# vpc-ccg/circminer

Measured on AMD Instinct MI355X. Metric: paired reads/sec (whole node), hg38 k=20, 2x150 bp; circ_report bit-exact, higher is better.
Workload: dtype int32/u8 (chain scores f64)

## Files before the change

### circminer_amd/csrc/cm_hot.hip

```cpp
#include <chrono>
#include <hip/hip_runtime.h>
#include <rocprim/device/device_radix_sort.hpp>

#include <algorithm>
#include <atomic>
#include <cstdarg>
#include <cstdio>
#include <cstdlib>
#include <cstring>
#include <string>
#include <functional>
#include <thread>
#include <vector>

#include "circminer_hot.h"
#include "cm_core.h"
#include "cm_aos.h"
#include "cm_index_build.h"

using cmc::Core;
using cmc::KCore;

namespace {

constexpr int MAX_SLOTS = 16;
constexpr uint32_t TILE_PAIRS = 1u << 20;
constexpr uint32_t TILE_PAIRS_MAX = 1u << 21;
constexpr int BLK = 256;
constexpr int BLK_CHAIN = 64;
#include "cm_dp_engine.h"

enum ProfClass { PC_NONE = -1, PC_SEED = 0, PC_CHAIN = 1, PC_PAIR = 2, PC_SCAN = 3, PC_HEAVY = 4, PC_ORDER = 5, PC_CHAIN_HEAVY = 6, PC_PREFETCH = 7, PC_COUNT = 8 };
enum Counter {
    CN_PROBES = 0 , CN_PAIR_ROUNDS = 3, CN_RERUN = 4 ,
    CN_FALL = 5, CN_FALL_2ND = 6,
    CN_CD_LANE = 8, CN_CD_PHASE = 13, CN_CD_WAVE = 16, CN_CD_EVENTS = 20, CN_CD_LEVELS = 21, CN_CD_PROBLEMS = 22, CN_CD_PASSES = 23, CN_CD_CELLS = 24,
    CN_CD_REGLOG = 25, CN_CD_BATCHES = 26, CN_CD_PRE_USED = 27, CN_CD_PRE_UNUSED = 28,
    CN_HP_ATTEMPT = 8, CN_HP_STRIDE = 8, CN_HP_UNPAIRED = 24, CN_HP_CHAINS = 25, CN_HP_SEQ_TASKS = 26, CN_HP_EARLY = 27, CN_HP_EARLY_FIRST = 28,
    CN_WORDS = 32
};
static_assert(CN_CD_CELLS < CN_WORDS && CN_HP_EARLY_FIRST < CN_WORDS && CN_HP_ATTEMPT + CN_HP_STRIDE + 5 < CN_HP_UNPAIRED, "d_counters has CN_WORDS words");
enum Pin {
    PIN_COLLECT_N = 0, PIN_COLLECT_ERR = 1,
    PIN_DEV_ERR = 0,
    PIN_POOL_ERR = 2,
    PIN_HEAVY_LOAD = 4,
    PIN_CELLS = 8,
    PIN_RERUN_N = 12, PIN_FALL_N = 14,
    PIN_WORDS = 16
};
constexpr size_t PIN_BYTES = PIN_WORDS * sizeof(unsigned long long);
static_assert(PIN_BYTES == 128 && PIN_FALL_N + 1 < PIN_WORDS && PIN_CELLS + 3 < PIN_RERUN_N, "the landing zone has 16 words");
struct ReadsDev {
    const uint8_t *seq1, *seq2;
    const uint64_t *off1, *off2;
};

__global__ void __launch_bounds__(BLK) k_seed(KCore kc, ReadsDev rd, const uint8_t *active, uint64_t pair0, uint32_t n_tile, int S,
                                              uint32_t *sstart, uint32_t *scnt, uint32_t *sraw, unsigned long long *counters) {
    const Core c = cmc::to_core(kc);
    __shared__ unsigned int sh[3];
    if (threadIdx.x < 3) sh[threadIdx.x] = 0;
    __syncthreads();
    const uint64_t q = (uint64_t)blockIdx.x * BLK + threadIdx.x;
    const uint64_t total = (uint64_t)n_tile * 4u * (uint64_t)S;
    if (q < total) {
        const uint32_t s = (uint32_t)(q % (uint64_t)S);
// ... 1827 lines not shown
struct StreamDef {
    hipStream_t Streams::*st;
    const char *name;
    StreamKind kind;
};
constexpr StreamDef STREAMS[] = {
    {&Streams::B, "main", BLOCKING},           {&Streams::B2, "heavy chains", BLOCKING},     {&Streams::C, "copy", NON_BLOCKING},
    {&Streams::P, "pairs", NON_BLOCKING_LOWEST}, {&Streams::P2, "heavy pairs", NON_BLOCKING}, {&Streams::R, "re-run", NON_BLOCKING},
    {&Streams::O, "pair ordering", NON_BLOCKING}, {&Streams::S, "seeding", NON_BLOCKING},
};
struct Events {
    hipEvent_t fork = nullptr, join = nullptr;
    hipEvent_t join_p = nullptr, tail = nullptr;
    hipEvent_t flags = nullptr;
    hipEvent_t staged = nullptr, retired = nullptr;
    hipEvent_t order[2] = {nullptr, nullptr};
    hipEvent_t seed[2] = {nullptr, nullptr};
    hipEvent_t first[2] = {nullptr, nullptr};
    hipEvent_t prep[2] = {nullptr, nullptr}, pair[2] = {nullptr, nullptr};
    hipEvent_t *begin() { return &fork; }
    hipEvent_t *end() { return begin() + sizeof(Events) / sizeof(hipEvent_t); }
};
static_assert(sizeof(Events) == 17 * sizeof(hipEvent_t), "Events holds events only");

}

struct cm_ctx {
    cm_params P{};
    unsigned id = 0;
    int teardown_errors = 0;
    Streams st;
    Events ev;
    std::vector<DevMem *> bufs[2];
    struct Rerun {
        bool deferred = false;
        cmc::KCore core;
        ReadsDev rd;
        uint64_t p0 = 0;
        uint32_t nt = 0;
        cm_chain *chains = nullptr;
        int32_t *nchain = nullptr, *high = nullptr;
        uint8_t *act_out = nullptr;
        int is_last = 0, cap2 = 0;
        size_t lds2 = 0;
        bool fall = false;
        size_t lds_heavy = 0;
        int str_cap = 0;
        unsigned fall_grid = 0;
    } rerun[2];
    bool pair_pending[2] = {false, false};
    int item_base = 0;
    bool pre_launched = false;
    bool pre_ready = false;
    int pre_slot = -1, pre_b = 0;
    uint64_t pre_gen = 0, pre_n = 0;
    uint32_t pre_nt = 0;
    BatchBuf<uint8_t> d_ones;
    uint64_t ones_cap = 0;
    unsigned long long *h_pin = nullptr;
    uint32_t h_pin_nt = 0;
    std::string err = "";
    Slot slots[MAX_SLOTS];
    uint64_t n_pairs = 0;
    ReadBufs rd;
    BatchBuf<cm_mapped_read> d_state;
    BatchBuf<uint8_t> d_active;
    BatchBuf<uint8_t> d_active_b;
    BatchBuf<int32_t> d_cat;
    int n_seeds = 0, max_len = 0;
    bool staged = false;
    uint64_t st_n_pairs = 0;
    ReadBufs st_rd;
    BatchBuf<cm_mapped_read> st_prior;
    bool st_has_prior = false;
    int st_max_len = 0;
    uint32_t tile = 0;
    SeedSet seed[2];
    ChainRecs rec[2];
    PairSetMem pair_mem;
    PairSet pset[2];
    PairSort sort;
    ChainWork dp;
    HeavyPipe hp;
    Collect col;
    BatchBuf<unsigned long long> d_lane_clk;
    BatchBuf<HRes> d_hres;
    BatchBuf<unsigned long long> d_type_hist;
    BatchBuf<unsigned long long> d_heavy_load;
    BatchBuf<cmc::MemoSpill> d_spill;
    CtxBuf<unsigned long long> d_pool_cursor;
    unsigned long long *pool_cursor(int s) const { return d_pool_cursor + s; }
    CtxBuf<int> d_err;
    CtxBuf<unsigned long long> d_counters;
    std::vector<unsigned long long> h_celloff;
    bool prof = false;
// ... 58 lines not shown
    m.cap = bytes;
    if (!m.listed) (m.listed = &c->bufs[L])->push_back(&m);
    return e;
}
void release(cm_ctx *c, Life l) {
    for (DevMem *m : c->bufs[l]) {
        dfree(c, *m);
        m->listed = nullptr;
    }
    c->bufs[l].clear();
}

void free_reads(cm_ctx *c) {
    if (c->st.C) report_hip(c, "hipStreamSynchronize(copy stream)", hipStreamSynchronize(c->st.C));
    release(c, BATCH);
    c->pset[0] = c->pset[1] = PairSet{};
    c->ones_cap = 0;
    c->pre_launched = c->pre_ready = false;
    c->staged = false;
    c->st_n_pairs = 0;
    c->n_pairs = 0;
    c->tile = 0;
}

static hipEvent_t take_event(cm_ctx *c) {
    hipEvent_t e = nullptr;
    if (!c->ev_free.empty()) {
        e = c->ev_free.back();
        c->ev_free.pop_back();
    } else (void)hipEventCreate(&e);
    return e;
}
struct Timer {
// ... 63 lines not shown
    if (!ctx->slots[slot].loaded) return fail(ctx, CM_ESTATE, "contig slot %d not loaded", slot);
    if (need_annot && !ctx->slots[slot].has_annot) return fail(ctx, CM_ESTATE, "annotation of slot %d not loaded", slot);
    return CM_OK;
}

ReadsDev reads_dev(const ReadBufs &r) { return ReadsDev{r.seq1_base + cmc::CM_STAGE_PAD, r.seq2_base + cmc::CM_STAGE_PAD, r.off1, r.off2}; }
ReadsDev current_reads(const cm_ctx *ctx) { return reads_dev(ctx->rd); }

constexpr unsigned HP_PLAN_GRID = 2048;
static bool heavy_pipeline() {
    static const bool v = !(getenv("CM_HEAVY_PIPELINE") && getenv("CM_HEAVY_PIPELINE")[0] == '0');
    return v;
}
static unsigned long long chain_light_w() {
    static const unsigned long long v = getenv("CM_CHAIN_LIGHT_W") ? strtoull(getenv("CM_CHAIN_LIGHT_W"), nullptr, 10) : 256ull;
    return v;
}
static unsigned int chain_light_cells() {
    static const unsigned int v = getenv("CM_CHAIN_LIGHT_CELLS") ? (unsigned)atoi(getenv("CM_CHAIN_LIGHT_CELLS")) : 96u;
    return v;
}

static int seed_classes(cm_ctx *ctx, uint64_t pair0, uint32_t n_tile, const uint8_t *act, int s, hipStream_t st, const ChainRecs *rb, bool defer = false) {
    const int S = ctx->n_seeds;
    const uint32_t n_prob = n_tile * 4u;
    if ((uint64_t)n_prob * (uint64_t)S == 0) return CM_OK;
    const SeedSet &sb = ctx->seed[s];
    Timer t(ctx, PC_ORDER, st);
    launch(ctx, PC_ORDER, k_chain_cls, dim3((n_prob + BLK - 1) / BLK), dim3(BLK), 0, st, sb.scnt, sb.sraw, S, n_prob, sb.cls4, defer ? sb.thigh : rb->high,
           chain_light_w(), chain_light_cells(), defer ? (int32_t *)nullptr : rb->nchain, defer ? (uint16_t *)nullptr : rb->resid, act, pair0);
// ... 753 lines not shown
    ctx->tile = tile;
    const size_t nprob = (size_t)tile * 4, nprobe = nprob * (size_t)(ctx->n_seeds ? ctx->n_seeds : 1);
    for (SeedSet &sd : ctx->seed) {
        HIPCHK(ctx, ensure(ctx, sd.sstart, nprobe * 4));
        HIPCHK(ctx, ensure(ctx, sd.scnt, nprobe * 4));
        HIPCHK(ctx, ensure(ctx, sd.sraw, nprobe * 4));
        HIPCHK(ctx, ensure(ctx, sd.celloff, (nprob + 2) * 8));
        HIPCHK(ctx, ensure(ctx, sd.bmax, (nprob / SCAN_ELEMS + 2) * 4));
        HIPCHK(ctx, ensure(ctx, sd.bsum, (nprob / SCAN_ELEMS + 2) * 8));
        HIPCHK(ctx, ensure(ctx, sd.cctr, CTR_WORDS * sizeof(unsigned int)));
        HIPCHK(ctx, ensure(ctx, sd.cblk, (size_t)N_CLS * (4 * (size_t)tile / CLS_T + 2) * sizeof(unsigned int)));
        HIPCHK(ctx, ensure(ctx, sd.cls4, (size_t)tile * 4));
        HIPCHK(ctx, ensure(ctx, sd.perm4, (size_t)tile * 4 * 4));
        HIPCHK(ctx, ensure(ctx, sd.thigh, (size_t)tile * 4 * sizeof(int32_t)));
    }
    for (ChainRecs &cr : ctx->rec) {
        HIPCHK(ctx, ensure(ctx, cr.chains, nprob * CM_BESTCHAINLIM * sizeof(cm_chain)));
        HIPCHK(ctx, ensure(ctx, cr.nchain, nprob * 4));
        HIPCHK(ctx, ensure(ctx, cr.high, nprob * 4));
        HIPCHK(ctx, ensure(ctx, cr.resid, (size_t)tile * 4 * sizeof(uint16_t)));
    }
    unsigned long long cap = (unsigned long long)nprob * 64ull;
    const unsigned long long worst = (unsigned long long)ctx->P.seed_lim * (unsigned long long)(ctx->n_seeds ? ctx->n_seeds : 1);
    if (cap < (8ull << 20)) cap = 8ull << 20;
    if (cap < worst) cap = worst;
    if (cap > ctx->dp.cells_cap || !ctx->dp.score) ctx->dp.cells_cap = cap;
    HIPCHK(ctx, ensure(ctx, ctx->dp.score, ctx->dp.cells_cap * sizeof(double)));
    HIPCHK(ctx, ensure(ctx, ctx->dp.prev, ctx->dp.cells_cap * sizeof(int32_t)));
    HIPCHK(ctx, ensure(ctx, ctx->sort.cls, (size_t)tile));
    PairSetMem &pm = ctx->pair_mem;
    HIPCHK(ctx, ensure(ctx, pm.perm, (size_t)tile * 4 * 2));
    HIPCHK(ctx, ensure(ctx, pm.hlist, (size_t)tile * 4 * 2));
    HIPCHK(ctx, ensure(ctx, ctx->d_hres, (size_t)HEAVY_GRID_MAX * (64 * sizeof(HRes) + HEAVY_SCRATCH)));
    if (heavy_pipeline()) {
        const size_t tc = getenv("CM_HP_TASKS_CAP") ? (size_t)std::max(1, atoi(getenv("CM_HP_TASKS_CAP"))) : std::max<size_t>((size_t)tile * 6, 4096);
        const size_t uc = getenv("CM_HP_UNP_CAP") ? (size_t)std::max(1, atoi(getenv("CM_HP_UNP_CAP"))) : std::max<size_t>((size_t)tile * 4, 4096);
        ctx->hp.tasks_cap = (uint32_t)tc;
        ctx->hp.unp_cap = (uint32_t)uc;
        HIPCHK(ctx, ensure(ctx, ctx->hp.pairs, (size_t)tile * sizeof(HPair)));
        HIPCHK(ctx, ensure(ctx, ctx->hp.list2, (size_t)tile * 4));
        HIPCHK(ctx, ensure(ctx, pm.hp_fall, (size_t)tile * 4 * 2));
        HIPCHK(ctx, ensure(ctx, pm.hp_fallctr, 2 * sizeof(unsigned int)));
        HIPCHK(ctx, ensure(ctx, ctx->hp.T, tc * sizeof(HTask)));
        HIPCHK(ctx, ensure(ctx, ctx->hp.tcls, tc));
        HIPCHK(ctx, ensure(ctx, ctx->hp.tperm, tc * 4));
        HIPCHK(ctx, ensure(ctx, ctx->hp.tblk, (size_t)N_CLS * (tc / CLS_T + 2) * sizeof(unsigned int)));
        HIPCHK(ctx, ensure(ctx, ctx->hp.tctr, CTR_WORDS * sizeof(unsigned int)));
        HIPCHK(ctx, ensure(ctx, ctx->hp.pre, tc * 4 * sizeof(cmc::PreDP)));
        HIPCHK(ctx, ensure(ctx, ctx->hp.q, tc * 4 * 4));
        HIPCHK(ctx, ensure(ctx, ctx->hp.res, tc * sizeof(HRes)));
        HIPCHK(ctx, ensure(ctx, ctx->hp.U, uc * sizeof(HUnp)));
        HIPCHK(ctx, ensure(ctx, ctx->hp.pre2, uc * 2 * sizeof(cmc::PreDP)));
        HIPCHK(ctx, ensure(ctx, ctx->hp.q2, uc * 2 * 4));
        HIPCHK(ctx, ensure(ctx, ctx->hp.lists, (size_t)HP_PLAN_GRID * HEAVY_LIST * 2));
        HIPCHK(ctx, ensure(ctx, ctx->hp.ctr, HC_WORDS * sizeof(unsigned int)));
    }
    {
        const uint32_t *before = pm.pair_err;
        HIPCHK(ctx, ensure(ctx, pm.pair_err, (size_t)tile * 4 * 2));
        if (pm.pair_err != before) HIPCHK(ctx, hipMemsetAsync(pm.pair_err, 0, (size_t)tile * 4 * 2, ctx->st.P));
    }
    HIPCHK(ctx, ensure(ctx, pm.retry_list, (size_t)tile * 4 * 2));
    HIPCHK(ctx, ensure(ctx, pm.retry_ctr, 4 * sizeof(unsigned int)));
    HIPCHK(ctx, ensure(ctx, ctx->d_heavy_load, sizeof(unsigned long long)));
    HIPCHK(ctx, ensure(ctx, ctx->d_spill, (size_t)RETRY_GRID * BLK_PAIR * RETRY_SPILL * sizeof(cmc::MemoSpill)));
    HIPCHK(ctx, ensure(ctx, pm.cls_ctr, 2 * CTR_WORDS * sizeof(unsigned int)));
    HIPCHK(ctx, ensure(ctx, ctx->sort.ctr2, CTR_WORDS * sizeof(unsigned int)));
    HIPCHK(ctx, ensure(ctx, ctx->sort.sub, (size_t)tile));
    HIPCHK(ctx, ensure(ctx, ctx->sort.perm1, (size_t)tile * 4));
    HIPCHK(ctx, ensure(ctx, ctx->sort.ctr3, CTR_WORDS * sizeof(unsigned int)));
    HIPCHK(ctx, ensure(ctx, ctx->sort.sub2, (size_t)tile));
    HIPCHK(ctx, ensure(ctx, ctx->sort.perm0, (size_t)tile * 4));
    HIPCHK(ctx, ensure(ctx, ctx->sort.blk_cnt, (size_t)N_CLS * (4 * (size_t)tile / CLS_T + 2) * sizeof(unsigned int)));
    if (getenv("CM_LANE_CLK")) {
#if defined(CM_DIAG)
        const size_t clk_words = 16 * 2 + 1;
#else
        const size_t clk_words = 1;
#endif
        HIPCHK(ctx, ensure(ctx, ctx->d_lane_clk, n * 8 * clk_words));
        HIPCHK(ctx, hipMemsetAsync(ctx->d_lane_clk, 0, n * 8 * clk_words, ctx->st.B));
    }
    unsigned long long pool = (unsigned long long)nprob * 2048ull;
    if (pool < (256ull << 20)) pool = 256ull << 20;
    if (pool > (8ull << 30)) pool = 8ull << 30;
    if (const char *e = getenv("CM_POOL_BYTES")) {
        const unsigned long long v = strtoull(e, nullptr, 10);
        if (v >= 4096 && !ctx->dp.pool) pool = v;
    }
    if (pool > ctx->dp.pool_bytes || !ctx->dp.pool) ctx->dp.pool_bytes = pool;
    HIPCHK(ctx, ensure(ctx, ctx->dp.pool, ctx->dp.pool_bytes));
    for (int b = 0; b < 2; ++b) {
        const size_t at = (size_t)b * tile;
        ctx->pset[b] = PairSet{pm.perm + at,       pm.hlist + at,      pm.cls_ctr + (size_t)b * CTR_WORDS,
                               pm.pair_err + at,   pm.retry_list + at, pm.retry_ctr + 2 * b,
                               pm.hp_fall ? pm.hp_fall + at : nullptr, pm.hp_fallctr ? pm.hp_fallctr + b : nullptr};
    }
    return CM_OK;
}

static int copy_reads(cm_ctx *ctx, const cm_reads *rd, hipStream_t st, ReadBufs &to) {
    const uint64_t n = rd->n_pairs;
    const size_t b1 = (size_t)rd->off1[n] - (size_t)rd->off1[0], b2 = (size_t)rd->off2[n] - (size_t)rd->off2[0];
    if (rd->off1[0] != 0 || rd->off2[0] != 0) return fail(ctx, CM_EINVAL, "read offsets must start at 0");
    const size_t pad = cmc::CM_STAGE_PAD;
    HIPCHK(ctx, ensure(ctx, to.seq1_base, b1 + 2 * pad));
    HIPCHK(ctx, ensure(ctx, to.seq2_base, b2 + 2 * pad));
// ... 3 lines not shown
    HIPCHK(ctx, hipMemsetAsync(to.seq1_base + pad + b1, 0, pad, st));
    HIPCHK(ctx, hipMemsetAsync(to.seq2_base, 0, pad, st));
    HIPCHK(ctx, hipMemsetAsync(to.seq2_base + pad + b2, 0, pad, st));
    if (b1) HIPCHK(ctx, hipMemcpyAsync(to.seq1_base + pad, rd->seq1, b1, hipMemcpyHostToDevice, st));
    if (b2) HIPCHK(ctx, hipMemcpyAsync(to.seq2_base + pad, rd->seq2, b2, hipMemcpyHostToDevice, st));
    HIPCHK(ctx, hipMemcpyAsync(to.off1, rd->off1, (n + 1) * sizeof(uint64_t), hipMemcpyHostToDevice, st));
    HIPCHK(ctx, hipMemcpyAsync(to.off2, rd->off2, (n + 1) * sizeof(uint64_t), hipMemcpyHostToDevice, st));
    return CM_OK;
}

int cm_reads_upload(cm_ctx *ctx, const cm_reads *rd, const cm_mapped_read *prior) {
    if (!ctx || !rd) return CM_EINVAL;
    HIPCHK(ctx, hipSetDevice(ctx->P.device));
    HIPCHK(ctx, hipStreamSynchronize(ctx->st.B));
    const uint64_t n = rd->n_pairs;
    ctx->pre_ready = false;
    ctx->n_pairs = 0;
    ctx->tile = 0;
    if (n == 0) {
        free_reads(ctx);
        return CM_OK;
    }
    int max_len = 0;
    int rc = check_reads(ctx, rd, &max_len);
    if (rc) return rc;
    if ((rc = copy_reads(ctx, rd, ctx->st.B, ctx->rd))) return rc;
    if ((rc = prepare_resident(ctx, n, max_len))) return rc;
    ctx->n_pairs = n;
    KCore k{};
    k.P = ctx->P;
    hipLaunchKernelGGL(k_init_state, dim3((unsigned)((n + BLK - 1) / BLK)), dim3(BLK), 0, ctx->st.B, k, ctx->d_state, ctx->d_active, ctx->d_cat, n);
// ... 1 lines not shown
        HIPCHK(ctx, hipMemcpyAsync(ctx->d_state, prior, n * sizeof(cm_mapped_read), hipMemcpyHostToDevice, ctx->st.B));
    }
    HIPCHK(ctx, hipStreamSynchronize(ctx->st.B));
    return CM_OK;
}

int cm_reads_stage(cm_ctx *ctx, const cm_reads *rd, const cm_mapped_read *prior) {
    if (!ctx || !rd) return CM_EINVAL;
    HIPCHK(ctx, hipSetDevice(ctx->P.device));
    if (rd->n_pairs == 0) return fail(ctx, CM_EINVAL, "cm_reads_stage: empty batch");
    int max_len = 0;
    int rc = check_reads(ctx, rd, &max_len);
    if (rc) return rc;
    HIPCHK(ctx, hipStreamSynchronize(ctx->st.C));
    ctx->staged = false;
    ctx->pre_launched = false;
    if ((rc = copy_reads(ctx, rd, ctx->st.C, ctx->st_rd))) return rc;
    ctx->st_has_prior = prior != nullptr;
    if (prior) {
        HIPCHK(ctx, ensure(ctx, ctx->st_prior, rd->n_pairs * sizeof(cm_mapped_read)));
        HIPCHK(ctx, hipMemcpyAsync(ctx->st_prior, prior, rd->n_pairs * sizeof(cm_mapped_read), hipMemcpyHostToDevice, ctx->st.C));
    }
    HIPCHK(ctx, hipEventRecord(ctx->ev.staged, ctx->st.C));
    ctx->st_n_pairs = rd->n_pairs;
    ctx->st_max_len = max_len;
    ctx->staged = true;
    return CM_OK;
}

int cm_reads_swap(cm_ctx *ctx) {
    if (!ctx) return CM_EINVAL;
    HIPCHK(ctx, hipSetDevice(ctx->P.device));
    if (!ctx->staged) return fail(ctx, CM_ESTATE, "cm_reads_swap: no staged batch");
    swap(ctx->rd, ctx->st_rd);
    ctx->staged = false;
    const uint64_t n = ctx->st_n_pairs;
    ctx->pre_ready = ctx->pre_launched;
    ctx->pre_launched = false;
    ctx->pre_n = n;
    ctx->n_pairs = 0;
    int rc = prepare_resident(ctx, n, ctx->st_max_len);
    if (rc) return rc;
    ctx->n_pairs = n;
    HIPCHK(ctx, hipStreamWaitEvent(ctx->st.B, ctx->ev.staged, 0));
    KCore k{};
    k.P = ctx->P;
    hipLaunchKernelGGL(k_init_state, dim3((unsigned)((n + BLK - 1) / BLK)), dim3(BLK), 0, ctx->st.B, k, ctx->d_state, ctx->d_active, ctx->d_cat, n);
    if (ctx->st_has_prior)
        HIPCHK(ctx, hipMemcpyAsync(ctx->d_state, ctx->st_prior, n * sizeof(cm_mapped_read), hipMemcpyDeviceToDevice, ctx->st.B));
    HIPCHK(ctx, hipEventRecord(ctx->ev.retired, ctx->st.B));
    HIPCHK(ctx, hipStreamWaitEvent(ctx->st.C, ctx->ev.retired, 0));
    HIPCHK(ctx, hipGetLastError());
    return CM_OK;
// ... 26 lines not shown
    bool fell = false;
    if (ctx->rerun[b].fall && (!wait || *(const volatile unsigned int *)(ctx->h_pin + PIN_FALL_N + b) != 0u)) {
        const int rc = launch_fall_back(ctx, b, ctx->st.R);
        if (rc) return rc;
        fell = true;
    }
    if (!wait || fell || *(const volatile unsigned int *)(ctx->h_pin + PIN_RERUN_N + b) != 0u) {
        const int rc = launch_rerun(ctx, b);
        if (rc) return rc;
    }
    HIPCHK(ctx, hipEventRecord(ctx->ev.pair[b], ctx->st.R));
    return CM_OK;
}

static int run_pair_tile(cm_ctx *ctx, const KCore &core, uint64_t p0, uint32_t nt, int is_last_round, const uint8_t *act_in, uint8_t *act_out,
                         const ChainRecs &rb, int b, bool same_tile_as_prev, bool defer) {
    const ReadsDev rd = current_reads(ctx);
    hipStream_t sp = ctx->st.P, sp2 = ctx->st.P2, sp3 = ctx->st.R;
    {
        int rc;
        if ((rc = settle_pair(ctx, b))) return rc;
        if (same_tile_as_prev && (rc = settle_pair(ctx, b ^ 1))) return rc;
    }
    hipStream_t so = ctx->st.O;
    HIPCHK(ctx, hipStreamWaitEvent(so, ctx->ev.prep[b], 0));
    if (same_tile_as_prev && ctx->pair_pending[b ^ 1]) HIPCHK(ctx, hipStreamWaitEvent(so, ctx->ev.pair[b ^ 1], 0));
    const PairSet &ps = ctx->pset[b];
    uint32_t *const perm = ps.perm, *const hlist = ps.hlist, *const pair_err = ps.pair_err;
    unsigned int *const cls_ctr = ps.cls_ctr, *const retry_ctr = ps.retry_ctr;
    constexpr int str_slack = 4;
    const int str_cap = ((ctx->max_len - ctx->P.kmer + ctx->P.band + str_slack + 7) / 8) * 8;
    constexpr unsigned slots_per_simd = 4;
    const size_t lds_bytes = (size_t)2 * lbuf_bytes(str_cap) * BLK_PAIR;
    const size_t lds_heavy = lds_bytes + HG * sizeof(HSlot);
    const int cap2 = std::min(((2 * ctx->max_len + 64 + 7) / 8) * 8, 1016);
    const size_t lds2 = (size_t)2 * lbuf_bytes(cap2) * BLK_PAIR;
    {
        static std::atomic<size_t> lim[3] = {{48u * 1024u}, {48u * 1024u}, {48u * 1024u}};
        const void *fn[3] = {(const void *)k_pair, (const void *)k_pair_rerun, (const void *)k_pair_heavy};
        const size_t want[3] = {lds_bytes, lds2, lds_heavy};
        for (int k = 0; k < 3; ++k)
// ... 137 lines not shown
    struct Item { uint64_t p0; uint32_t nt; int r; };
    std::vector<Item> items;
    const uint64_t n_tiles = (ctx->n_pairs + ctx->tile - 1) / ctx->tile;
    const bool round_major = n_tiles >= 2;
    auto tile_nt = [&](uint64_t t) { return (uint32_t)((ctx->n_pairs - t * ctx->tile < ctx->tile) ? ctx->n_pairs - t * ctx->tile : ctx->tile); };
    if (round_major) {
        for (int r = 0; r < n_rounds; ++r)
            for (uint64_t t = 0; t < n_tiles; ++t) items.push_back(Item{t * ctx->tile, tile_nt(t), r});
    } else {
        for (uint64_t t = 0; t < n_tiles; ++t)
            for (int r = 0; r < n_rounds; ++r) items.push_back(Item{t * ctx->tile, tile_nt(t), r});
    }
    const int n_items = (int)items.size();
    std::vector<int> tiles_of_round((size_t)n_rounds, 0);
    const bool use_pre = ctx->pre_ready && slots[0] == ctx->pre_slot && ctx->slots[slots[0]].gen == ctx->pre_gen && ctx->n_pairs == ctx->pre_n &&
                         items[0].nt == ctx->pre_nt && (ctx->item_base & 1) == ctx->pre_b;
    ctx->pre_ready = ctx->pre_launched = false;
    if (use_pre) ++ctx->launches[PC_PREFETCH];
    const ReadsDev rd_cur = current_reads(ctx);
    auto prep_flags = [&](int i) -> const uint8_t * {
        const int r = items[i].r;
        return round_major ? A[r & 1] : ((r == 0) ? A[0] : A[(r - 1) & 1]);
    };
    std::vector<char> seeded((size_t)n_items, 0);
    bool pre_seeded = false;
    const bool early_ok = round_major;
    auto issue_seed_early = [&](int i) -> int {
        HIPCHK(ctx, hipStreamWaitEvent(ctx->st.S, ctx->ev.flags, 0));
        if (n_tiles == 2 && i >= 2) HIPCHK(ctx, hipStreamWaitEvent(ctx->st.S, ctx->ev.first[(ctx->item_base + i) & 1], 0));
        const ChainRecs &rbe = ctx->rec[(ctx->item_base + i) & 1];
        const int e = run_seed_tile(ctx, make_core(ctx, ctx->slots[slots[items[i].r]]), rd_cur, items[i].p0, items[i].nt, prep_flags(i), i & 1, ctx->st.S, &rbe, true);
        seeded[(size_t)i] = 1;
        return e;
    };
    auto issue_seed = [&](int i, hipStream_t st) -> int {
        const int b = (ctx->item_base + i) & 1;
        int e;
        if ((e = settle_pair(ctx, b))) return e;
        if (ctx->pair_pending[b]) HIPCHK(ctx, hipStreamWaitEvent(st, ctx->ev.pair[b], 0));
        const ChainRecs &rbi = ctx->rec[b];
        e = run_seed_tile(ctx, make_core(ctx, ctx->slots[slots[items[i].r]]), rd_cur, items[i].p0, items[i].nt, prep_flags(i), i & 1, st, &rbi);
        seeded[(size_t)i] = 1;
        return e;
    };
    for (int i = 0; i < n_items; ++i) {
        const uint64_t p0 = items[i].p0;
        const uint32_t nt = items[i].nt;
        const int r = items[i].r, b = (ctx->item_base + i) & 1;
        const Slot &sl = ctx->slots[slots[r]];
        const KCore core = make_core(ctx, sl);
        const ChainRecs &rb = ctx->rec[b];
        const uint8_t *act_prep = prep_flags(i);
        auto ahead = [&]() -> int {
            if (i + 1 >= n_items || seeded[(size_t)i + 1]) return CM_OK;
            if (early_ok) return issue_seed_early(i + 1);
            const int bn = (ctx->item_base + i + 1) & 1;
            if (ctx->rerun[bn].deferred && hipEventQuery(ctx->ev.first[bn]) != hipSuccess) {
                (void)hipGetLastError();
                return CM_OK;
            }
            return issue_seed(i + 1, ctx->st.S);
        };
        auto late = [&]() -> int { return (i + 1 < n_items && !seeded[(size_t)i + 1]) ? issue_seed(i + 1, ctx->st.S) : CM_OK; };
        if (i == n_items - 1 && prefetch && !pre_seeded) {
            const Slot &sl0 = ctx->slots[slots[0]];
            const uint32_t nt0 = tile_for(ctx->st_n_pairs);
            const ReadsDev rd_next = reads_dev(ctx->st_rd);
            HIPCHK(ctx, hipStreamWaitEvent(ctx->st.S, ctx->ev.staged, 0));
            if ((rc = run_seed_tile(ctx, make_core(ctx, sl0), rd_next, 0, nt0, ctx->d_ones, n_items & 1, ctx->st.S, nullptr))) return rc;
            pre_seeded = true;
        }
        if (use_pre && i == 0) {
            if ((rc = ahead())) return rc;
        } else {
            if (!seeded[(size_t)i] && (rc = issue_seed(i, ctx->st.B))) return rc;
            if ((rc = settle_pair(ctx, b))) return rc;
            if (ctx->pair_pending[b]) {
                HIPCHK(ctx, hipStreamWaitEvent(ctx->st.B, ctx->ev.pair[b], 0));
                ctx->pair_pending[b] = false;
            }
            HIPCHK(ctx, hipEventRecord(ctx->ev.flags, ctx->st.B));
            if ((rc = run_chain_tile(ctx, core, rd_cur, p0, nt, sl.chain_parallel_ok, act_prep, rb, i & 1, ahead))) return rc;
            HIPCHK(ctx, hipEventRecord(ctx->ev.prep[b], ctx->st.B));
        }
        const int is_last = (r == n_rounds - 1) ? (last_is_final != 0) : 0;
        const bool same_tile = i > 0 && items[i - 1].p0 == p0;
        if ((rc = run_pair_tile(ctx, core, p0, nt, is_last, A[r & 1], A[(r + 1) & 1], rb, b, same_tile, round_major))) return rc;
        if ((rc = late())) return rc;
        ++*items_done;
        if (++tiles_of_round[(size_t)r] == (int)n_tiles) ++*rounds_done;
    }
    ctx->item_base = (ctx->item_base + n_items) & 1;
    *items_done = 0;
    if (prefetch) {
        const int b = ctx->item_base;
        const Slot &sl = ctx->slots[slots[0]];
        const KCore core = make_core(ctx, sl);
        const uint32_t nt = tile_for(ctx->st_n_pairs);
        HIPCHK(ctx, hipStreamWaitEvent(ctx->st.B, ctx->ev.staged, 0));
        if ((rc = settle_pair(ctx, b))) return rc;
        if (ctx->pair_pending[b]) {
            HIPCHK(ctx, hipStreamWaitEvent(ctx->st.B, ctx->ev.pair[b], 0));
            ctx->pair_pending[b] = false;
        }
        const ChainRecs &rbn = ctx->rec[b];
        const ReadsDev rd_next = reads_dev(ctx->st_rd);
        if (pre_seeded) {
            HIPCHK(ctx, hipStreamWaitEvent(ctx->st.B, ctx->ev.seed[n_items & 1], 0));
            if ((rc = seed_classes(ctx, 0, nt, ctx->d_ones, n_items & 1, ctx->st.B, &rbn))) return rc;
        } else if ((rc = run_seed_tile(ctx, core, rd_next, 0, nt, ctx->d_ones, n_items & 1, ctx->st.B, &rbn))) return rc;
        if ((rc = run_chain_tile(ctx, core, rd_next, 0, nt, sl.chain_parallel_ok, ctx->d_ones, rbn, n_items & 1))) return rc;
        HIPCHK(ctx, hipEventRecord(ctx->ev.prep[b], ctx->st.B));
        ctx->pre_launched = true;
        ctx->pre_slot = slots[0];
        ctx->pre_gen = sl.gen;
        ctx->pre_b = b;
        ctx->pre_nt = nt;
    }
    if ((rc = settle_pair(ctx, ctx->item_base, false)) || (rc = settle_pair(ctx, ctx->item_base ^ 1, false))) return rc;
    HIPCHK(ctx, hipEventRecord(ctx->ev.tail, ctx->st.R));
    HIPCHK(ctx, hipStreamWaitEvent(ctx->st.B, ctx->ev.tail, 0));
    ctx->pair_pending[0] = ctx->pair_pending[1] = false;
    if (n_rounds & 1) swap(ctx->d_active, ctx->d_active_b);
    *rounds_done = 0;
    return CM_OK;
}

int cm_map_rounds(cm_ctx *ctx, const int *slots, int n_rounds, int last_is_final) {
    if (!ctx || (n_rounds > 0 && !slots) || n_rounds < 0) return CM_EINVAL;
    int rc;
    for (int r = 0; r < n_rounds; ++r)
        if ((rc = check_slot(ctx, slots[r], true))) return rc;
    HIPCHK(ctx, hipSetDevice(ctx->P.device));
    if (ctx->n_pairs == 0 || n_rounds == 0) return CM_OK;
    int items_done = 0, rounds_done = 0;
    rc = map_rounds_issue(ctx, slots, n_rounds, last_is_final, &items_done, &rounds_done);
    if (rc == CM_OK) return rc;
    for (const StreamDef &d : STREAMS)
        if (d.st != &Streams::C) (void)hipStreamSynchronize(ctx->st.*d.st);
    ctx->rerun[0].deferred = ctx->rerun[1].deferred = false;
    ctx->seed[0].cls_deferred = ctx->seed[1].cls_deferred = false;
    ctx->item_base = (ctx->item_base + items_done) & 1;
    if (rounds_done & 1) swap(ctx->d_active, ctx->d_active_b);
    ctx->pair_pending[0] = ctx->pair_pending[1] = false;
    ctx->pre_ready = ctx->pre_launched = false;
    return rc;
}

int cm_map_round(cm_ctx *ctx, int slot, int is_last_round) { return cm_map_rounds(ctx, &slot, 1, is_last_round); }

int cm_sync(cm_ctx *ctx) {
    if (!ctx) return CM_EINVAL;
    HIPCHK(ctx, hipSetDevice(ctx->P.device));
    HIPCHK(ctx, hipStreamSynchronize(ctx->st.B));
    HIPCHK(ctx, hipStreamSynchronize(ctx->st.C));
    return check_dev_err(ctx);
}

int cm_reads_reset(cm_ctx *ctx) {
    if (!ctx) return CM_EINVAL;
// ... 245 lines not shown
}

int cm_prof_reset(cm_ctx *ctx) {
    if (!ctx) return CM_EINVAL;
    HIPCHK(ctx, hipSetDevice(ctx->P.device));
    HIPCHK(ctx, hipStreamSynchronize(ctx->st.B));
    for (auto &r : ctx->recs) {
        ctx->ev_free.push_back(r.a);
        ctx->ev_free.push_back(r.b);
    }
    ctx->recs.clear();
    for (int i = 0; i < PC_COUNT; ++i) {
        ctx->ms[i] = 0;
        ctx->launches[i] = 0;
    }
    HIPCHK(ctx, hipMemsetAsync(ctx->d_counters, 0, CN_WORDS * sizeof(unsigned long long), ctx->st.B));
    HIPCHK(ctx, hipStreamSynchronize(ctx->st.B));
    return CM_OK;
}

int cm_prof_get(cm_ctx *ctx, double ms[8], uint64_t launches[8]) {
    if (!ctx || !ms || !launches) return CM_EINVAL;
    HIPCHK(ctx, hipSetDevice(ctx->P.device));
    HIPCHK(ctx, hipStreamSynchronize(ctx->st.B));
    for (auto &r : ctx->recs) {
        float t = 0;
        if (hipEventElapsedTime(&t, r.a, r.b) == hipSuccess) ctx->ms[r.cls] += (double)t;
        ctx->ev_free.push_back(r.a);
        ctx->ev_free.push_back(r.b);
    }
    ctx->recs.clear();
    for (int i = 0; i < PC_COUNT; ++i) {
        ms[i] = ctx->ms[i];
        launches[i] = ctx->launches[i];
    }
    return CM_OK;
}

int cm_prof_counters(cm_ctx *ctx, uint64_t c[8]) {
    if (!ctx || !c) return CM_EINVAL;
    HIPCHK(ctx, hipSetDevice(ctx->P.device));
    unsigned long long h[8] = {0, 0, 0, 0, 0, 0, 0, 0};
    HIPCHK(ctx, hipMemcpyAsync(h, ctx->d_counters, sizeof h, hipMemcpyDeviceToHost, ctx->st.B));
    HIPCHK(ctx, hipStreamSynchronize(ctx->st.B));
    for (int i = 0; i < 8; ++i) c[i] = h[i];
    return CM_OK;
}

}
```

Baseline: 29.67 million.

## Add third chain-record set and prefetch second tile of next batch

Moves from two rotating chain-record and pair sets to three, indexed by item_base modulo 6, so seeding and chaining of a later tile can run while pairing of earlier tiles is still in flight. The cross-batch prefetch now seeds and chains a second tile of the staged batch as well as the first, which the next map_rounds call can consume. This aims to hide more of the inter-batch seam and tile dependencies. It costs more device memory and more event/settle bookkeeping. If allocation fails or CM_CHAIN_SETS=2 is set, it falls back to two sets.

```diff
diff --git a/circminer_amd/csrc/cm_hot.hip b/circminer_amd/csrc/cm_hot.hip
--- a/circminer_amd/csrc/cm_hot.hip
+++ b/circminer_amd/csrc/cm_hot.hip
@@ -34,6 +34,7 @@
 enum Counter {
     CN_PROBES = 0 , CN_PAIR_ROUNDS = 3, CN_RERUN = 4 ,
     CN_FALL = 5, CN_FALL_2ND = 6,
+    CN_PRE_SECOND = 7,
     CN_CD_LANE = 8, CN_CD_PHASE = 13, CN_CD_WAVE = 16, CN_CD_EVENTS = 20, CN_CD_LEVELS = 21, CN_CD_PROBLEMS = 22, CN_CD_PASSES = 23, CN_CD_CELLS = 24,
     CN_CD_REGLOG = 25, CN_CD_BATCHES = 26, CN_CD_PRE_USED = 27, CN_CD_PRE_UNUSED = 28,
     CN_HP_ATTEMPT = 8, CN_HP_STRIDE = 8, CN_HP_UNPAIRED = 24, CN_HP_CHAINS = 25, CN_HP_SEQ_TASKS = 26, CN_HP_EARLY = 27, CN_HP_EARLY_FIRST = 28,
@@ -45,12 +46,15 @@
     PIN_DEV_ERR = 0,
     PIN_POOL_ERR = 2,
     PIN_HEAVY_LOAD = 4,
+    PIN_RERUN_N = 5,
     PIN_CELLS = 8,
-    PIN_RERUN_N = 12, PIN_FALL_N = 14,
+    PIN_FALL_N = 12,
     PIN_WORDS = 16
 };
+constexpr int MAX_SETS = 3;
 constexpr size_t PIN_BYTES = PIN_WORDS * sizeof(unsigned long long);
-static_assert(PIN_BYTES == 128 && PIN_FALL_N + 1 < PIN_WORDS && PIN_CELLS + 3 < PIN_RERUN_N, "the landing zone has 16 words");
+static_assert(PIN_BYTES == 128 && PIN_HEAVY_LOAD < PIN_RERUN_N && PIN_RERUN_N + MAX_SETS <= PIN_CELLS && PIN_CELLS + 3 < PIN_FALL_N &&
+              PIN_FALL_N + MAX_SETS <= PIN_WORDS, "the landing zone has 16 words");
 struct ReadsDev {
     const uint8_t *seq1, *seq2;
     const uint64_t *off1, *off2;
@@ -1908,14 +1912,14 @@
     hipEvent_t join_p = nullptr, tail = nullptr;
     hipEvent_t flags = nullptr;
     hipEvent_t staged = nullptr, retired = nullptr;
-    hipEvent_t order[2] = {nullptr, nullptr};
+    hipEvent_t order[MAX_SETS] = {};
     hipEvent_t seed[2] = {nullptr, nullptr};
-    hipEvent_t first[2] = {nullptr, nullptr};
-    hipEvent_t prep[2] = {nullptr, nullptr}, pair[2] = {nullptr, nullptr};
+    hipEvent_t first[MAX_SETS] = {};
+    hipEvent_t prep[MAX_SETS] = {}, pair[MAX_SETS] = {};
     hipEvent_t *begin() { return &fork; }
     hipEvent_t *end() { return begin() + sizeof(Events) / sizeof(hipEvent_t); }
 };
-static_assert(sizeof(Events) == 17 * sizeof(hipEvent_t), "Events holds events only");
+static_assert(sizeof(Events) == (9 + 4 * MAX_SETS) * sizeof(hipEvent_t), "Events holds events only");
 
 }
 
@@ -1941,14 +1945,21 @@
         size_t lds_heavy = 0;
         int str_cap = 0;
         unsigned fall_grid = 0;
-    } rerun[2];
-    bool pair_pending[2] = {false, false};
+    } rerun[MAX_SETS];
+    bool pair_pending[MAX_SETS] = {};
+    int n_sets = 2;
+    bool third_set_refused = false;
     int item_base = 0;
-    bool pre_launched = false;
-    bool pre_ready = false;
-    int pre_slot = -1, pre_b = 0;
+    int set_of(int i) const { return (item_base + i + 6) % n_sets; }
+    bool pre_launched = false, pre2_launched = false;
+    bool pre_ready = false, pre2_ready = false;
+    int pre_slot = -1, pre_b = 0, pre2_b = 0;
     uint64_t pre_gen = 0, pre_n = 0;
     uint32_t pre_nt = 0;
+    uint64_t pre2_p0 = 0;
+    uint32_t pre2_nt = 0;
+    uint64_t pre2_taken = 0;
+    void drop_prepared() { pre_launched = pre_ready = pre2_launched = pre2_ready = false; }
     BatchBuf<uint8_t> d_ones;
     uint64_t ones_cap = 0;
     unsigned long long *h_pin = nullptr;
@@ -1970,9 +1981,9 @@
     int st_max_len = 0;
     uint32_t tile = 0;
     SeedSet seed[2];
-    ChainRecs rec[2];
+    ChainRecs rec[MAX_SETS];
     PairSetMem pair_mem;
-    PairSet pset[2];
+    PairSet pset[MAX_SETS];
     PairSort sort;
     ChainWork dp;
     HeavyPipe hp;
@@ -2061,9 +2072,9 @@
 void free_reads(cm_ctx *c) {
     if (c->st.C) report_hip(c, "hipStreamSynchronize(copy stream)", hipStreamSynchronize(c->st.C));
     release(c, BATCH);
-    c->pset[0] = c->pset[1] = PairSet{};
+    for (PairSet &ps : c->pset) ps = PairSet{};
     c->ones_cap = 0;
-    c->pre_launched = c->pre_ready = false;
+    c->drop_prepared();
     c->staged = false;
     c->st_n_pairs = 0;
     c->n_pairs = 0;
@@ -2157,6 +2168,10 @@
 }
 static unsigned long long chain_light_w() {
     static const unsigned long long v = getenv("CM_CHAIN_LIGHT_W") ? strtoull(getenv("CM_CHAIN_LIGHT_W"), nullptr, 10) : 256ull;
+    return v;
+}
+static bool third_set_wanted() {
+    static const bool v = !(getenv("CM_CHAIN_SETS") && atoi(getenv("CM_CHAIN_SETS")) == 2);
     return v;
 }
 static unsigned int chain_light_cells() {
@@ -2940,7 +2955,8 @@
         HIPCHK(ctx, ensure(ctx, sd.perm4, (size_t)tile * 4 * 4));
         HIPCHK(ctx, ensure(ctx, sd.thigh, (size_t)tile * 4 * sizeof(int32_t)));
     }
-    for (ChainRecs &cr : ctx->rec) {
+    for (int b = 0; b < 2; ++b) {
+        ChainRecs &cr = ctx->rec[b];
         HIPCHK(ctx, ensure(ctx, cr.chains, nprob * CM_BESTCHAINLIM * sizeof(cm_chain)));
         HIPCHK(ctx, ensure(ctx, cr.nchain, nprob * 4));
         HIPCHK(ctx, ensure(ctx, cr.high, nprob * 4));
@@ -2955,8 +2971,8 @@
     HIPCHK(ctx, ensure(ctx, ctx->dp.prev, ctx->dp.cells_cap * sizeof(int32_t)));
     HIPCHK(ctx, ensure(ctx, ctx->sort.cls, (size_t)tile));
     PairSetMem &pm = ctx->pair_mem;
-    HIPCHK(ctx, ensure(ctx, pm.perm, (size_t)tile * 4 * 2));
-    HIPCHK(ctx, ensure(ctx, pm.hlist, (size_t)tile * 4 * 2));
+    HIPCHK(ctx, ensure(ctx, pm.perm, (size_t)tile * 4 * MAX_SETS));
+    HIPCHK(ctx, ensure(ctx, pm.hlist, (size_t)tile * 4 * MAX_SETS));
     HIPCHK(ctx, ensure(ctx, ctx->d_hres, (size_t)HEAVY_GRID_MAX * (64 * sizeof(HRes) + HEAVY_SCRATCH)));
     if (heavy_pipeline()) {
         const size_t tc = getenv("CM_HP_TASKS_CAP") ? (size_t)std::max(1, atoi(getenv("CM_HP_TASKS_CAP"))) : std::max<size_t>((size_t)tile * 6, 4096);
@@ -2965,8 +2981,8 @@
         ctx->hp.unp_cap = (uint32_t)uc;
         HIPCHK(ctx, ensure(ctx, ctx->hp.pairs, (size_t)tile * sizeof(HPair)));
         HIPCHK(ctx, ensure(ctx, ctx->hp.list2, (size_t)tile * 4));
-        HIPCHK(ctx, ensure(ctx, pm.hp_fall, (size_t)tile * 4 * 2));
-        HIPCHK(ctx, ensure(ctx, pm.hp_fallctr, 2 * sizeof(unsigned int)));
+        HIPCHK(ctx, ensure(ctx, pm.hp_fall, (size_t)tile * 4 * MAX_SETS));
+        HIPCHK(ctx, ensure(ctx, pm.hp_fallctr, MAX_SETS * sizeof(unsigned int)));
         HIPCHK(ctx, ensure(ctx, ctx->hp.T, tc * sizeof(HTask)));
         HIPCHK(ctx, ensure(ctx, ctx->hp.tcls, tc));
         HIPCHK(ctx, ensure(ctx, ctx->hp.tperm, tc * 4));
@@ -2983,14 +2999,14 @@
     }
     {
         const uint32_t *before = pm.pair_err;
-        HIPCHK(ctx, ensure(ctx, pm.pair_err, (size_t)tile * 4 * 2));
-        if (pm.pair_err != before) HIPCHK(ctx, hipMemsetAsync(pm.pair_err, 0, (size_t)tile * 4 * 2, ctx->st.P));
-    }
-    HIPCHK(ctx, ensure(ctx, pm.retry_list, (size_t)tile * 4 * 2));
-    HIPCHK(ctx, ensure(ctx, pm.retry_ctr, 4 * sizeof(unsigned int)));
+        HIPCHK(ctx, ensure(ctx, pm.pair_err, (size_t)tile * 4 * MAX_SETS));
+        if (pm.pair_err != before) HIPCHK(ctx, hipMemsetAsync(pm.pair_err, 0, (size_t)tile * 4 * MAX_SETS, ctx->st.P));
+    }
+    HIPCHK(ctx, ensure(ctx, pm.retry_list, (size_t)tile * 4 * MAX_SETS));
+    HIPCHK(ctx, ensure(ctx, pm.retry_ctr, 2 * MAX_SETS * sizeof(unsigned int)));
     HIPCHK(ctx, ensure(ctx, ctx->d_heavy_load, sizeof(unsigned long long)));
     HIPCHK(ctx, ensure(ctx, ctx->d_spill, (size_t)RETRY_GRID * BLK_PAIR * RETRY_SPILL * sizeof(cmc::MemoSpill)));
-    HIPCHK(ctx, ensure(ctx, pm.cls_ctr, 2 * CTR_WORDS * sizeof(unsigned int)));
+    HIPCHK(ctx, ensure(ctx, pm.cls_ctr, MAX_SETS * CTR_WORDS * sizeof(unsigned int)));
     HIPCHK(ctx, ensure(ctx, ctx->sort.ctr2, CTR_WORDS * sizeof(unsigned int)));
     HIPCHK(ctx, ensure(ctx, ctx->sort.sub, (size_t)tile));
     HIPCHK(ctx, ensure(ctx, ctx->sort.perm1, (size_t)tile * 4));
@@ -3016,7 +3032,20 @@
     }
     if (pool > ctx->dp.pool_bytes || !ctx->dp.pool) ctx->dp.pool_bytes = pool;
     HIPCHK(ctx, ensure(ctx, ctx->dp.pool, ctx->dp.pool_bytes));
-    for (int b = 0; b < 2; ++b) {
+    if (!third_set_wanted()) ctx->third_set_refused = true;
+    if (!ctx->third_set_refused) {
+        ChainRecs &cr = ctx->rec[2];
+        if (ensure(ctx, cr.chains, nprob * CM_BESTCHAINLIM * sizeof(cm_chain)) != hipSuccess || ensure(ctx, cr.nchain, nprob * 4) != hipSuccess ||
+            ensure(ctx, cr.high, nprob * 4) != hipSuccess || ensure(ctx, cr.resid, (size_t)tile * 4 * sizeof(uint16_t)) != hipSuccess) {
+            (void)hipGetLastError();
+            dfree(ctx, cr.chains), dfree(ctx, cr.nchain), dfree(ctx, cr.high), dfree(ctx, cr.resid);
+            ctx->third_set_refused = true;
+        }
+    }
+    const int n_sets = ctx->third_set_refused ? 2 : 3;
+    if (n_sets != ctx->n_sets) ctx->drop_prepared();
+    ctx->n_sets = n_sets;
+    for (int b = 0; b < MAX_SETS; ++b) {
         const size_t at = (size_t)b * tile;
         ctx->pset[b] = PairSet{pm.perm + at,       pm.hlist + at,      pm.cls_ctr + (size_t)b * CTR_WORDS,
                                pm.pair_err + at,   pm.retry_list + at, pm.retry_ctr + 2 * b,
@@ -3050,7 +3079,7 @@
     HIPCHK(ctx, hipSetDevice(ctx->P.device));
     HIPCHK(ctx, hipStreamSynchronize(ctx->st.B));
     const uint64_t n = rd->n_pairs;
-    ctx->pre_ready = false;
+    ctx->pre_ready = ctx->pre2_ready = false;
     ctx->n_pairs = 0;
     ctx->tile = 0;
     if (n == 0) {
@@ -3082,7 +3111,7 @@
     if (rc) return rc;
     HIPCHK(ctx, hipStreamSynchronize(ctx->st.C));
     ctx->staged = false;
-    ctx->pre_launched = false;
+    ctx->pre_launched = ctx->pre2_launched = false;
     if ((rc = copy_reads(ctx, rd, ctx->st.C, ctx->st_rd))) return rc;
     ctx->st_has_prior = prior != nullptr;
     if (prior) {
@@ -3104,7 +3133,8 @@
     ctx->staged = false;
     const uint64_t n = ctx->st_n_pairs;
     ctx->pre_ready = ctx->pre_launched;
-    ctx->pre_launched = false;
+    ctx->pre2_ready = ctx->pre_launched && ctx->pre2_launched;
+    ctx->pre_launched = ctx->pre2_launched = false;
     ctx->pre_n = n;
     ctx->n_pairs = 0;
     int rc = prepare_resident(ctx, n, ctx->st_max_len);
@@ -3161,17 +3191,17 @@
 }
 
 static int run_pair_tile(cm_ctx *ctx, const KCore &core, uint64_t p0, uint32_t nt, int is_last_round, const uint8_t *act_in, uint8_t *act_out,
-                         const ChainRecs &rb, int b, bool same_tile_as_prev, bool defer) {
+                         const ChainRecs &rb, int b, int b_prev, bool same_tile_as_prev, bool defer) {
     const ReadsDev rd = current_reads(ctx);
     hipStream_t sp = ctx->st.P, sp2 = ctx->st.P2, sp3 = ctx->st.R;
     {
         int rc;
         if ((rc = settle_pair(ctx, b))) return rc;
-        if (same_tile_as_prev && (rc = settle_pair(ctx, b ^ 1))) return rc;
+        if (same_tile_as_prev && (rc = settle_pair(ctx, b_prev))) return rc;
     }
     hipStream_t so = ctx->st.O;
     HIPCHK(ctx, hipStreamWaitEvent(so, ctx->ev.prep[b], 0));
-    if (same_tile_as_prev && ctx->pair_pending[b ^ 1]) HIPCHK(ctx, hipStreamWaitEvent(so, ctx->ev.pair[b ^ 1], 0));
+    if (same_tile_as_prev && ctx->pair_pending[b_prev]) HIPCHK(ctx, hipStreamWaitEvent(so, ctx->ev.pair[b_prev], 0));
     const PairSet &ps = ctx->pset[b];
     uint32_t *const perm = ps.perm, *const hlist = ps.hlist, *const pair_err = ps.pair_err;
     unsigned int *const cls_ctr = ps.cls_ctr, *const retry_ctr = ps.retry_ctr;
@@ -3339,30 +3369,39 @@
     const int n_items = (int)items.size();
     std::vector<int> tiles_of_round((size_t)n_rounds, 0);
     const bool use_pre = ctx->pre_ready && slots[0] == ctx->pre_slot && ctx->slots[slots[0]].gen == ctx->pre_gen && ctx->n_pairs == ctx->pre_n &&
-                         items[0].nt == ctx->pre_nt && (ctx->item_base & 1) == ctx->pre_b;
-    ctx->pre_ready = ctx->pre_launched = false;
+                         items[0].nt == ctx->pre_nt && ctx->set_of(0) == ctx->pre_b;
+    const bool use_pre2 = use_pre && ctx->pre2_ready && round_major && items[1].r == 0 && items[1].p0 == ctx->pre2_p0 && items[1].nt == ctx->pre2_nt &&
+                          ctx->set_of(1) == ctx->pre2_b;
+    ctx->drop_prepared();
     if (use_pre) ++ctx->launches[PC_PREFETCH];
+    if (use_pre2) ++ctx->pre2_taken;
     const ReadsDev rd_cur = current_reads(ctx);
     auto prep_flags = [&](int i) -> const uint8_t * {
         const int r = items[i].r;
         return round_major ? A[r & 1] : ((r == 0) ? A[0] : A[(r - 1) & 1]);
     };
     std::vector<char> seeded((size_t)n_items, 0);
+    if (use_pre2) seeded[1] = 1;
     bool pre_seeded = false;
+    auto behind_pair = [&](hipStream_t st, int s) -> int {
+        const int e = settle_pair(ctx, s);
+        if (e) return e;
+        if (ctx->pair_pending[s]) HIPCHK(ctx, hipStreamWaitEvent(st, ctx->ev.pair[s], 0));
+        return CM_OK;
+    };
     const bool early_ok = round_major;
     auto issue_seed_early = [&](int i) -> int {
         HIPCHK(ctx, hipStreamWaitEvent(ctx->st.S, ctx->ev.flags, 0));
-        if (n_tiles == 2 && i >= 2) HIPCHK(ctx, hipStreamWaitEvent(ctx->st.S, ctx->ev.first[(ctx->item_base + i) & 1], 0));
-        const ChainRecs &rbe = ctx->rec[(ctx->item_base + i) & 1];
+        if (n_tiles == 2 && i >= 2) HIPCHK(ctx, hipStreamWaitEvent(ctx->st.S, ctx->ev.first[ctx->set_of(i - 2)], 0));
+        const ChainRecs &rbe = ctx->rec[ctx->set_of(i)];
         const int e = run_seed_tile(ctx, make_core(ctx, ctx->slots[slots[items[i].r]]), rd_cur, items[i].p0, items[i].nt, prep_flags(i), i & 1, ctx->st.S, &rbe, true);
         seeded[(size_t)i] = 1;
         return e;
     };
     auto issue_seed = [&](int i, hipStream_t st) -> int {
-        const int b = (ctx->item_base + i) & 1;
+        const int b = ctx->set_of(i);
         int e;
-        if ((e = settle_pair(ctx, b))) return e;
-        if (ctx->pair_pending[b]) HIPCHK(ctx, hipStreamWaitEvent(st, ctx->ev.pair[b], 0));
+        if ((e = behind_pair(st, b)) || (e = behind_pair(st, ctx->set_of(i - 2)))) return e;
         const ChainRecs &rbi = ctx->rec[b];
         e = run_seed_tile(ctx, make_core(ctx, ctx->slots[slots[items[i].r]]), rd_cur, items[i].p0, items[i].nt, prep_flags(i), i & 1, st, &rbi);
         seeded[(size_t)i] = 1;
@@ -3371,7 +3410,7 @@
     for (int i = 0; i < n_items; ++i) {
         const uint64_t p0 = items[i].p0;
         const uint32_t nt = items[i].nt;
-        const int r = items[i].r, b = (ctx->item_base + i) & 1;
+        const int r = items[i].r, b = ctx->set_of(i);
         const Slot &sl = ctx->slots[slots[r]];
         const KCore core = make_core(ctx, sl);
         const ChainRecs &rb = ctx->rec[b];
@@ -3379,11 +3418,11 @@
         auto ahead = [&]() -> int {
             if (i + 1 >= n_items || seeded[(size_t)i + 1]) return CM_OK;
             if (early_ok) return issue_seed_early(i + 1);
-            const int bn = (ctx->item_base + i + 1) & 1;
-            if (ctx->rerun[bn].deferred && hipEventQuery(ctx->ev.first[bn]) != hipSuccess) {
-                (void)hipGetLastError();
-                return CM_OK;
-            }
+            for (const int bn : {ctx->set_of(i + 1), ctx->set_of(i - 1)})
+                if (ctx->rerun[bn].deferred && hipEventQuery(ctx->ev.first[bn]) != hipSuccess) {
+                    (void)hipGetLastError();
+                    return CM_OK;
+                }
             return issue_seed(i + 1, ctx->st.S);
         };
         auto late = [&]() -> int { return (i + 1 < n_items && !seeded[(size_t)i + 1]) ? issue_seed(i + 1, ctx->st.S) : CM_OK; };
@@ -3395,57 +3434,72 @@
             if ((rc = run_seed_tile(ctx, make_core(ctx, sl0), rd_next, 0, nt0, ctx->d_ones, n_items & 1, ctx->st.S, nullptr))) return rc;
             pre_seeded = true;
         }
-        if (use_pre && i == 0) {
+        if ((use_pre && i == 0) || (use_pre2 && i == 1)) {
             if ((rc = ahead())) return rc;
         } else {
             if (!seeded[(size_t)i] && (rc = issue_seed(i, ctx->st.B))) return rc;
-            if ((rc = settle_pair(ctx, b))) return rc;
-            if (ctx->pair_pending[b]) {
-                HIPCHK(ctx, hipStreamWaitEvent(ctx->st.B, ctx->ev.pair[b], 0));
-                ctx->pair_pending[b] = false;
-            }
+            if ((rc = behind_pair(ctx->st.B, b)) || (rc = behind_pair(ctx->st.B, ctx->set_of(i - 2)))) return rc;
             HIPCHK(ctx, hipEventRecord(ctx->ev.flags, ctx->st.B));
             if ((rc = run_chain_tile(ctx, core, rd_cur, p0, nt, sl.chain_parallel_ok, act_prep, rb, i & 1, ahead))) return rc;
             HIPCHK(ctx, hipEventRecord(ctx->ev.prep[b], ctx->st.B));
         }
         const int is_last = (r == n_rounds - 1) ? (last_is_final != 0) : 0;
         const bool same_tile = i > 0 && items[i - 1].p0 == p0;
-        if ((rc = run_pair_tile(ctx, core, p0, nt, is_last, A[r & 1], A[(r + 1) & 1], rb, b, same_tile, round_major))) return rc;
+        if ((rc = run_pair_tile(ctx, core, p0, nt, is_last, A[r & 1], A[(r + 1) & 1], rb, b, ctx->set_of(i - 1), same_tile, round_major))) return rc;
         if ((rc = late())) return rc;
         ++*items_done;
         if (++tiles_of_round[(size_t)r] == (int)n_tiles) ++*rounds_done;
     }
-    ctx->item_base = (ctx->item_base + n_items) & 1;
+    ctx->item_base = (ctx->item_base + n_items) % 6;
     *items_done = 0;
     if (prefetch) {
-        const int b = ctx->item_base;
+        const int b = ctx->set_of(0);
         const Slot &sl = ctx->slots[slots[0]];
         const KCore core = make_core(ctx, sl);
         const uint32_t nt = tile_for(ctx->st_n_pairs);
+        const uint64_t p2 = nt;
+        const uint32_t nt2 = (uint32_t)std::min<uint64_t>(ctx->st_n_pairs - p2, nt);
+#ifndef CM_PREFETCH_SECOND
+#define CM_PREFETCH_SECOND 1
+#endif
+        const bool second = CM_PREFETCH_SECOND && ctx->n_sets >= 3 && nt2 > 0;
+        const int s1 = n_items & 1, s2 = (n_items + 1) & 1;
         HIPCHK(ctx, hipStreamWaitEvent(ctx->st.B, ctx->ev.staged, 0));
-        if ((rc = settle_pair(ctx, b))) return rc;
-        if (ctx->pair_pending[b]) {
-            HIPCHK(ctx, hipStreamWaitEvent(ctx->st.B, ctx->ev.pair[b], 0));
-            ctx->pair_pending[b] = false;
-        }
+        if ((rc = behind_pair(ctx->st.B, b))) return rc;
         const ChainRecs &rbn = ctx->rec[b];
         const ReadsDev rd_next = reads_dev(ctx->st_rd);
         if (pre_seeded) {
-            HIPCHK(ctx, hipStreamWaitEvent(ctx->st.B, ctx->ev.seed[n_items & 1], 0));
-            if ((rc = seed_classes(ctx, 0, nt, ctx->d_ones, n_items & 1, ctx->st.B, &rbn))) return rc;
-        } else if ((rc = run_seed_tile(ctx, core, rd_next, 0, nt, ctx->d_ones, n_items & 1, ctx->st.B, &rbn))) return rc;
-        if ((rc = run_chain_tile(ctx, core, rd_next, 0, nt, sl.chain_parallel_ok, ctx->d_ones, rbn, n_items & 1))) return rc;
+            HIPCHK(ctx, hipStreamWaitEvent(ctx->st.B, ctx->ev.seed[s1], 0));
+            if ((rc = seed_classes(ctx, 0, nt, ctx->d_ones, s1, ctx->st.B, &rbn))) return rc;
+        } else if ((rc = run_seed_tile(ctx, core, rd_next, 0, nt, ctx->d_ones, s1, ctx->st.B, &rbn))) return rc;
+        auto seed_second = [&]() -> int {
+            if (!second) return CM_OK;
+            HIPCHK(ctx, hipStreamWaitEvent(ctx->st.S, ctx->ev.staged, 0));
+            return run_seed_tile(ctx, core, rd_next, p2, nt2, ctx->d_ones, s2, ctx->st.S, &ctx->rec[ctx->set_of(1)], true);
+        };
+        if ((rc = run_chain_tile(ctx, core, rd_next, 0, nt, sl.chain_parallel_ok, ctx->d_ones, rbn, s1, seed_second))) return rc;
         HIPCHK(ctx, hipEventRecord(ctx->ev.prep[b], ctx->st.B));
         ctx->pre_launched = true;
         ctx->pre_slot = slots[0];
         ctx->pre_gen = sl.gen;
         ctx->pre_b = b;
         ctx->pre_nt = nt;
-    }
-    if ((rc = settle_pair(ctx, ctx->item_base, false)) || (rc = settle_pair(ctx, ctx->item_base ^ 1, false))) return rc;
+        if (second) {
+            const int b2 = ctx->set_of(1);
+            if ((rc = behind_pair(ctx->st.B, b2))) return rc;
+            if ((rc = run_chain_tile(ctx, core, rd_next, p2, nt2, sl.chain_parallel_ok, ctx->d_ones, ctx->rec[b2], s2))) return rc;
+            HIPCHK(ctx, hipEventRecord(ctx->ev.prep[b2], ctx->st.B));
+            ctx->pre2_launched = true;
+            ctx->pre2_b = b2;
+            ctx->pre2_p0 = p2;
+            ctx->pre2_nt = nt2;
+        }
+    }
+    for (int k = ctx->n_sets; k >= 1; --k)
+        if ((rc = settle_pair(ctx, ctx->set_of(-k), false))) return rc;
     HIPCHK(ctx, hipEventRecord(ctx->ev.tail, ctx->st.R));
     HIPCHK(ctx, hipStreamWaitEvent(ctx->st.B, ctx->ev.tail, 0));
-    ctx->pair_pending[0] = ctx->pair_pending[1] = false;
+    for (bool &pp : ctx->pair_pending) pp = false;
     if (n_rounds & 1) swap(ctx->d_active, ctx->d_active_b);
     *rounds_done = 0;
     return CM_OK;
@@ -3463,12 +3517,12 @@
     if (rc == CM_OK) return rc;
     for (const StreamDef &d : STREAMS)
         if (d.st != &Streams::C) (void)hipStreamSynchronize(ctx->st.*d.st);
-    ctx->rerun[0].deferred = ctx->rerun[1].deferred = false;
+    for (cm_ctx::Rerun &q : ctx->rerun) q.deferred = false;
     ctx->seed[0].cls_deferred = ctx->seed[1].cls_deferred = false;
-    ctx->item_base = (ctx->item_base + items_done) & 1;
+    ctx->item_base = (ctx->item_base + items_done) % 6;
     if (rounds_done & 1) swap(ctx->d_active, ctx->d_active_b);
-    ctx->pair_pending[0] = ctx->pair_pending[1] = false;
-    ctx->pre_ready = ctx->pre_launched = false;
+    for (bool &pp : ctx->pair_pending) pp = false;
+    ctx->drop_prepared();
     return rc;
 }
 
@@ -3744,6 +3798,7 @@
         ctx->ms[i] = 0;
         ctx->launches[i] = 0;
     }
+    ctx->pre2_taken = 0;
     HIPCHK(ctx, hipMemsetAsync(ctx->d_counters, 0, CN_WORDS * sizeof(unsigned long long), ctx->st.B));
     HIPCHK(ctx, hipStreamSynchronize(ctx->st.B));
     return CM_OK;
@@ -3774,7 +3829,8 @@
     HIPCHK(ctx, hipMemcpyAsync(h, ctx->d_counters, sizeof h, hipMemcpyDeviceToHost, ctx->st.B));
     HIPCHK(ctx, hipStreamSynchronize(ctx->st.B));
     for (int i = 0; i < 8; ++i) c[i] = h[i];
-    return CM_OK;
-}
-
-}
+    c[CN_PRE_SECOND] = ctx->pre2_taken;
+    return CM_OK;
+}
+
+}
```

Result: slower. 27.05 million (-8.8%).
